# dkohlsdorf/audio_pattern_discovery

Hardware: AMD Instinct MI355X
Metric: DTW cell-updates/sec (whole node) (higher is better)
Workload: dtype f32

## Files before the change

### audio_pattern_discovery_amd/csrc/apd_internal.h

```cpp
#pragma once
#include <hip/hip_runtime.h>
#include <stdint.h>

#include <iterator>
#include <map>
#include <set>
#include <string>
#include <type_traits>
#include <utility>
#include <vector>

#include "../../include/apd.h"

struct apd_context;
namespace apd {

constexpr int kTile = 16;
constexpr int kSlotsPerTile = kTile * kTile;
constexpr int kWave = 64;

struct BandSpec {
    float pct;
    uint32_t explicit_band;
    int use_explicit;
    float ins, del, mat;
};

struct AlignLaunch {
    const float *d_frames;
    uint32_t frames_bytes;
    const uint32_t *d_seq_off;
    const float *d_seq_nmax;
    const uint4 *d_tiles;
    uint32_t n_tiles;
    uint32_t n_seq;
    uint32_t dim, dpad;
    BandSpec band;
    float *d_slab;
    const uint32_t *d_nonfinite;
    uint32_t w_max;
    uint32_t n_max;
    int variant;
    int hybrid;
    int strict;
    float tau;
};

constexpr int kKernelDims[] = {8, 10, 13, 16, 20, 26};
constexpr bool is_kernel_dim(uint32_t d) { for (int k : kKernelDims) if ((uint32_t)k == d) return true; return false; }
constexpr uint32_t kernel_dim(uint32_t d) { for (int k : kKernelDims) if ((uint32_t)k >= d) return (uint32_t)k; return d; }
constexpr int max_cells_per_lane(uint32_t d) { return d <= 13 ? 9 : (d <= 16 ? 7 : 5); }
constexpr int max_strip_columns(uint32_t d) { return d <= 10 ? 13 : (d <= 13 ? 11 : max_cells_per_lane(d)); }

struct KernelGeom {
    enum Family : uint8_t { Generic, Systolic, Wide, Strip, BandedStrip, SharedColumns };
    Family family = Generic;
    uint8_t lanes_or_waves = 0;
    uint8_t cells = 0;

    constexpr int encode() const
    {
        constexpr int base[] = {0, 0, 10000, 20000, 30000, 40000};
        return family == Generic ? 0 : base[family] + lanes_or_waves * 100 + cells;
    }
    static constexpr KernelGeom decode(int key)
    {
        const Family f = key >= 100 && key < 10000 ? Systolic : key >= 10000 && key < 20000 ? Wide
                       : key >= 20000 && key < 30000 ? Strip : key >= 30000 && key < 40000 ? BandedStrip
                       : key >= 40000 && key < 50000 ? SharedColumns : Generic;
        if (f == Generic) return KernelGeom{};
        return KernelGeom{f, (uint8_t)((key % 10000) / 100), (uint8_t)(key % 100)};
    }
    constexpr uint32_t lanes_per_pair() const
    {
        return family == Systolic || family == SharedColumns ? lanes_or_waves : family == Wide ? 64u * lanes_or_waves : 64u;
    }
    constexpr uint32_t capacity() const { return (family == Wide ? 64u : 1u) * lanes_or_waves * cells; }
    constexpr bool operator==(KernelGeom o) const { return family == o.family && lanes_or_waves == o.lanes_or_waves && cells == o.cells; }
    constexpr bool operator<(KernelGeom o) const { return encode() < o.encode(); }
};

#define APD_SYSTOLIC_GEOMS(X) X(8, 5) X(8, 7) X(8, 9) X(16, 2) X(16, 3) X(16, 5) X(16, 7) X(16, 9) X(32, 5) X(32, 7) X(32, 9) \
                              X(64, 3) X(64, 5) X(64, 7) X(64, 9)
#define APD_WIDE_GEOMS(X) X(2, 5) X(2, 7) X(2, 9) X(4, 5) X(4, 7) X(4, 9) X(8, 5) X(8, 7) X(8, 9)
#define APD_STRIP_GEOMS(X) X(1, 3) X(1, 5) X(1, 7) X(1, 9) X(1, 11) X(1, 13) X(2, 3) X(2, 5) X(2, 7) X(2, 9) X(2, 11) X(2, 13) \
                           X(4, 3) X(4, 5) X(4, 7) X(4, 9) X(4, 11) X(4, 13)
#define APD_BANDED_STRIP_GEOMS(X) X(1, 5) X(1, 9) X(4, 5) X(4, 9)
#define APD_SHARED_COLUMN_GEOMS(X) X(16, 9)

#define APD_SYSTOLIC_ENTRY_(A, B) KernelGeom{KernelGeom::Systolic, A, B},
#define APD_WIDE_ENTRY_(A, B) KernelGeom{KernelGeom::Wide, A, B},
#define APD_STRIP_ENTRY_(A, B) KernelGeom{KernelGeom::Strip, A, B},
#define APD_BANDED_STRIP_ENTRY_(A, B) KernelGeom{KernelGeom::BandedStrip, A, B},
#define APD_SHARED_COLUMN_ENTRY_(A, B) KernelGeom{KernelGeom::SharedColumns, A, B},
constexpr KernelGeom kSystolicGeoms[] = {APD_SYSTOLIC_GEOMS(APD_SYSTOLIC_ENTRY_)};
constexpr KernelGeom kWideGeoms[] = {APD_WIDE_GEOMS(APD_WIDE_ENTRY_)};
constexpr KernelGeom kStripGeoms[] = {APD_STRIP_GEOMS(APD_STRIP_ENTRY_)};
constexpr KernelGeom kBandedStripGeoms[] = {APD_BANDED_STRIP_GEOMS(APD_BANDED_STRIP_ENTRY_)};
constexpr KernelGeom kSharedColumnGeoms[] = {APD_SHARED_COLUMN_GEOMS(APD_SHARED_COLUMN_ENTRY_)};
#undef APD_SYSTOLIC_ENTRY_
#undef APD_WIDE_ENTRY_
#undef APD_STRIP_ENTRY_
#undef APD_BANDED_STRIP_ENTRY_
#undef APD_SHARED_COLUMN_ENTRY_

template <class F, size_t... I>
bool with_kernel_dim_(uint32_t dim, F &&f, std::index_sequence<I...>)
{
    return ((dim == (uint32_t)kKernelDims[I] ? (f(std::integral_constant<int, kKernelDims[I]>{}), true) : false) || ...);
}
template <class F>
bool with_kernel_dim(uint32_t dim, F &&f) { return with_kernel_dim_(dim, f, std::make_index_sequence<std::size(kKernelDims)>{}); }

constexpr bool geom_instantiated(KernelGeom g, uint32_t dim)
{
    if (g.family == KernelGeom::Generic) return true;
    if (!is_kernel_dim(dim)) return false;
    const bool strip = g.family == KernelGeom::Strip;
    if (g.cells > (strip ? max_strip_columns(dim) : max_cells_per_lane(dim))) return false;
    auto on = [g](const auto &list) { for (KernelGeom e : list) if (e == g) return true; return false; };
    return g.family == KernelGeom::Systolic ? on(kSystolicGeoms) : g.family == KernelGeom::Wide ? on(kWideGeoms)
         : g.family == KernelGeom::SharedColumns ? on(kSharedColumnGeoms) : strip ? on(kStripGeoms) : on(kBandedStripGeoms);
}
template <size_t N>
constexpr bool geoms_round_trip(const KernelGeom (&list)[N])
{
    for (KernelGeom g : list) if (!(KernelGeom::decode(g.encode()) == g)) return false;
    return true;
}
static_assert(geoms_round_trip(kSystolicGeoms) && geoms_round_trip(kWideGeoms) && geoms_round_trip(kStripGeoms) &&
                  geoms_round_trip(kBandedStripGeoms) && geoms_round_trip(kSharedColumnGeoms), "a listed geometry has no integer code of its own");

__host__ __device__ constexpr int sweep_result_offset(int rows, int cols, int w) { return (cols - 1) - (rows - 1) + w; }
__host__ __device__ constexpr int sweep_capture_step(int rows, int cols, int w, int c)
{
    return (rows - 1) + sweep_result_offset(rows, cols, w) / c;
}
__host__ __device__ constexpr int sweep_steps_needed(int rows, int cols, int w, int c) { return sweep_capture_step(rows, cols, w, c) + 1; }
static_assert(sweep_result_offset(1000, 1024, 66) == 90 && sweep_capture_step(1000, 1024, 66, 9) == 1009 &&
                  sweep_steps_needed(1000, 1024, 66, 9) == 1010, "cfg 3's shape, rows the shorter sequence: lane 10 ends the sweep");
static_assert(sweep_steps_needed(1024, 1000, 66, 9) == 1028, "the same pair with the longer sequence as rows: u* = 42, lane 4");
static_assert(sweep_capture_step(40, 72, 34, 9) == 39 + 7 && (2 * 34 + 1 + 8) / 9 == 8,
              "|n - m| = w - 2: u* = 2w - 2 sits in the last active lane, nothing is cut at the end");
static_assert(sweep_steps_needed(2, 2, 2, 2) == 3 && sweep_steps_needed(72, 40, 34, 9) == 72, "smallest pair; u* = 2: lane 0");

constexpr int shared_column_unroll(int c) { return (c + 1) % 2 == 0 ? c + 1 : 2 * (c + 1); }
constexpr int shared_column_ring_min(int g, int c) { return (g - 1) * (c - 1) + 1 + 2 * shared_column_unroll(c); }
constexpr int shared_column_ring_frames(int g, int c) { return (shared_column_ring_min(g, c) + 16 + 7) / 8 * 8; }
constexpr uint32_t shared_column_slack(KernelGeom g)
{
    return (uint32_t)(shared_column_ring_frames(g.lanes_or_waves, g.cells) - shared_column_ring_min(g.lanes_or_waves, g.cells));
}
inline uint32_t host_w(const BandSpec &b, uint32_t n, uint32_t m);
inline bool shared_columns_qualify(const std::vector<uint32_t> &lens, uint32_t tile_a, uint32_t tile_b, const BandSpec &band,
                                   uint32_t slack)
{
    const uint32_t n_seq = (uint32_t)lens.size();
    for (uint32_t sa = 0; sa < (uint32_t)kTile; sa += 4)
        for (uint32_t sb = 0; sb < (uint32_t)kTile; sb += 4) {
            uint32_t lo = 0xFFFFFFFFu, hi = 0;
            for (uint32_t i = 0; i < 16; ++i) {
                const uint32_t a = tile_a * kTile + sa + i / 4, b = tile_b * kTile + sb + i % 4;
                if (!(a < b && b < n_seq) || lens[a] < 2 || lens[b] < 2) continue;
                const uint32_t w = host_w(band, lens[a], lens[b]);
                lo = w < lo ? w : lo;
                hi = w > hi ? w : hi;
            }
            if (hi > lo && hi - lo > slack) return false;
        }
    return true;
}

constexpr uint64_t strip_lds_bytes(uint32_t dim, uint32_t ppw, bool banded, uint32_t rows)
{
    const uint64_t dp = (dim + 4) & ~3u;
    return 4 * ((ppw == 1 ? 128 : 64) * dp + (uint64_t)ppw * (banded ? 2 : 1) * (rows + 4) + 16);
}

constexpr uint32_t kPathMaxOffsets = 20480;
__host__ __device__ constexpr uint32_t path_cells_per_lane(uint32_t w) { return (2 * w + 1 + 63) / 64 < 2 ? 2u : (2 * w + 1 + 63) / 64; }
inline uint64_t path_dir_words(uint32_t n, uint32_t m, uint32_t w)
{
    if (n < 2 || m < 2) return 0;
    return ((uint64_t)n + 63) * ((path_cells_per_lane(w) + 15) / 16) * 64;
}
struct PathPair {
    uint32_t px, py;
    uint64_t dir_off;
    uint64_t step_off;
};
struct PathLaunch {
    const float *d_frames;
    const uint32_t *d_seq_off;
    uint32_t dim, dpad;
    BandSpec band;
    const PathPair *d_pairs;
    uint32_t n_pairs;
    uint32_t *d_dirs;
    apd_path_step *d_steps;
    uint32_t *d_len;
    float *d_scores;
};
hipError_t launch_path_sweep(const PathLaunch &L, uint32_t c_max, hipStream_t stream);
hipError_t launch_path_trace(const PathLaunch &L, hipStream_t stream);

constexpr uint32_t kSpotMaxQuery = 16384;
constexpr uint32_t kSpotMaxStream = 0xFFFF0000u;
constexpr uint32_t kSpotRegisterRows = 4;
constexpr uint32_t spot_rows_per_lane(uint32_t n) { return (n + 63) / 64; }
constexpr uint32_t spot_row_class(uint32_t dim, uint32_t n)
{
    return is_kernel_dim(dim) && spot_rows_per_lane(n) <= kSpotRegisterRows ? spot_rows_per_lane(n) : 0u;
}
struct SpotPair {
    uint32_t px, py;
    uint32_t out;
    uint32_t pad;
    uint64_t curve_off;
};
struct SpotLaunch {
    const float *d_frames;
    const uint32_t *d_seq_off;
    uint32_t dim, dpad;
    float ins, del, mat;
    const SpotPair *d_pairs;
    uint32_t n_pairs;
    float *d_cost;
    uint32_t *d_start;
    apd_spot_best *d_best;
};
size_t spot_lds_bytes(uint32_t rows_per_lane);
hipError_t launch_spot(const SpotLaunch &L, uint32_t rt, uint32_t r_max, hipStream_t stream);

hipError_t launch_align(const AlignLaunch &L, KernelGeom g, hipStream_t stream, std::string &err, int *status);
hipError_t launch_generic_fallback(const AlignLaunch &L, hipStream_t stream, bool *fits);
bool generic_fallback_fits(uint32_t w_max);

struct TileClass { KernelGeom geom; uint32_t first, count, w_max, n_max; };
void plan_tile_classes(const std::vector<uint64_t> &offsets, uint32_t n_seq, const std::vector<uint2> &tiles, const BandSpec &band,
                       uint32_t dim, int variant, bool fast_ok, bool uniform_pen, bool fast_shift, std::vector<TileClass> &classes,
                       std::vector<uint4> &flat);
hipError_t launch_pad(const float *d_src, float *d_dst, const uint32_t *d_seq_off, const uint32_t *d_src_off, uint32_t n_seq,
                      uint64_t n_frames_padded, uint32_t src_dim, uint32_t dim, uint32_t dpad, uint32_t *d_flags, float *d_seq_nmax,
                      hipStream_t stream);
hipError_t launch_unpack(const float *d_gathered, float *d_out, const uint32_t *d_order, uint32_t n_seq, uint32_t world,
                         uint64_t slab_floats, const uint32_t *d_flags, uint32_t *d_status, hipStream_t stream);
hipError_t launch_selftest(int *d_result, hipStream_t stream);
hipError_t launch_join_flags(uint32_t *d_flags_out, const uint32_t *d_flags_a, const uint32_t *d_flags_b, hipStream_t stream);
hipError_t launch_unpack_cross(const float *d_slab, float *d_fs, float *d_sf, const uint32_t *d_order, uint32_t n_seq, uint32_t n0,
                               uint32_t n_first, bool swapped, const uint32_t *d_flags, uint32_t *d_status, hipStream_t stream);
hipError_t launch_cross_linkage(const float *d_fs, const float *d_sf, uint32_t n_first, uint32_t n_second, const uint32_t *d_members,
                                const uint32_t *d_set_off, uint32_t n_sets, float *d_link, uint32_t *d_nearest, float *d_nearest_linkage,
                                hipStream_t stream);
hipError_t launch_sqrt_sweep(uint32_t first, uint64_t count, unsigned long long *d_out, hipStream_t stream);
constexpr float kFeatureFloor = 0x1p-40f;
constexpr float kFeatureBound = 0x1p60f;

struct DeviceBuf {
    void *ptr = nullptr;
    size_t bytes = 0;
    DeviceBuf() = default;
    DeviceBuf(DeviceBuf &&o) noexcept : ptr(o.ptr), bytes(o.bytes) { o.ptr = nullptr; o.bytes = 0; }
    DeviceBuf &operator=(DeviceBuf &&o) noexcept { std::swap(ptr, o.ptr); std::swap(bytes, o.bytes); return *this; }
    ~DeviceBuf() { reset(); }
    hipError_t reset() { const hipError_t e = ptr ? hipFree(ptr) : hipSuccess; ptr = nullptr; bytes = 0; return e; }
    hipError_t alloc(size_t n)
    {
        if (hipError_t e = reset(); e != hipSuccess) return e;
        if (hipError_t e = hipMalloc(&ptr, n); e != hipSuccess) { ptr = nullptr; return e; }
        bytes = n;
        return hipSuccess;
    }
    hipError_t reserve(size_t n) { return ptr && bytes >= n ? hipSuccess : alloc(n); }
    template <class T> T *as() const { return static_cast<T *>(ptr); }
    explicit operator bool() const { return ptr != nullptr; }
};

struct ContextChild {
    apd_context *ctx = nullptr;
    virtual void release_device() = 0;
    virtual ~ContextChild() = default;
};
int destroy_child(ContextChild *child);

int device_select(apd_context *ctx, const float *d_x, uint64_t len, uint64_t k, float *value);
uint64_t percentile_index(uint64_t len, float perc);

inline uint32_t host_band_from_pct(float pct, uint32_t len)
{
    float p = pct * (float)len;
    if (!(p > 0.0f)) return 0;
    if (p >= 4294967040.0f) return 0xFFFFFFFFu;
    return (uint32_t)p;
}
inline uint32_t host_w(const BandSpec &b, uint32_t n, uint32_t m)
{
    uint32_t mx = n > m ? n : m, gap = n > m ? n - m : m - n;
// ... 85 lines not shown
```

### audio_pattern_discovery_amd/csrc/dtw_systolic.h

```cpp
#pragma once
#include <type_traits>

#ifndef APD_ABLATE
#define APD_ABLATE 0
#endif

#include "dtw_common.h"

namespace apd {

typedef float apd_f32x4 __attribute__((ext_vector_type(4)));
constexpr uint32_t kNoFrame = 0xFFFFFF00u;

template <int D>
__device__ __forceinline__ void load_frame(float (&dst)[D], __amdgpu_buffer_rsrc_t rsrc, uint32_t byte_off)
{
    constexpr int DP4 = (D + 3) / 4;
#pragma unroll
    for (int q = 0; q < DP4; ++q) {
        const apd_f32x4 t = __builtin_bit_cast(apd_f32x4, __builtin_amdgcn_raw_buffer_load_b128(rsrc, byte_off + 16u * q, 0, 0));
        if (4 * q + 0 < D) dst[4 * q + 0] = t.x;
        if (4 * q + 1 < D) dst[4 * q + 1] = t.y;
        if (4 * q + 2 < D) dst[4 * q + 2] = t.z;
        if (4 * q + 3 < D) dst[4 * q + 3] = t.w;
// ... 255 lines not shown
            const apd_f32x4 t = *reinterpret_cast<const apd_f32x4 *>(p + 4 * q);
            if (4 * q + 0 < DN) dst[4 * q + 0] = t.x;
            if (4 * q + 1 < DN) dst[4 * q + 1] = t.y;
            if (4 * q + 2 < DN) dst[4 * q + 2] = t.z;
            if (4 * q + 3 < DN) dst[4 * q + 3] = t.w;
        }
    };
    constexpr int NX = HYBRID ? 1 : 2;
    float xs[NX][DN];
    read_row(xs[0], 0 - gl);
#pragma unroll
    for (int k = 0; k < DN; ++k) xs[NX - 1][k] = (NX == 1) ? xs[0][k] : 0.0f;
    constexpr bool PIPE = (APD_ABLATE & 32) != 0;
    float dn[C];
#pragma unroll
    for (int c = 0; c < C; ++c) dn[c] = (PIPE && !HYBRID && c < C - 1) ? frame_dist_strict<D, DN>(xs[0], yf[c]) : 0.0f;

    auto advance_window = [&](int q) __attribute__((always_inline)) {
        const int r = q % S, e = (r + C) % S;
#pragma unroll
        for (int k = 0; k < (HYBRID ? DN : D); ++k) {
            if (APD_ABLATE & 4) { yf[e][k] = yf[(r + 1) % S][k] + yf[e][k]; continue; }
            yf[e][k] = MASKED_FETCH ? dpp_move<(G == 8) ? 0x101 : 0x130>(yf[(r + 1) % S][k], yf[e][k])
                                    : group_from_upper<G>(yf[(r + 1) % S][k], yf[e][k], gl);
        }
    };
    auto macro_steps = [&](int tau_begin, int tau_end, auto slow_tag) __attribute__((always_inline)) {
        constexpr bool SLOW = decltype(slow_tag)::value;
        uint32_t yo_cur = kNoFrame, yo_cap = kNoFrame, yo_step = 0u;
        if (!SLOW && gl == G - 1) {
            yo_cap = b_off + (uint32_t)(m - 1) * FB;
            yo_cur = min(b_off + (uint32_t)(tau_begin + ((HYBRID && !MASKED_FETCH) ? 1 : 0) + (C - 1) * G - w) * FB, yo_cap);
            yo_step = FB;
        }
        auto fetch_column = [&](float (&dst)[DN], int t) __attribute__((always_inline)) {
            if (APD_ABLATE & 8) return;
            if (SLOW) {
                const int jt = t + 1 + (C - 1) * G - w;
                const uint32_t yo = b_off + (uint32_t)((jt >= 1) ? (min(jt, m) - 1) : (HYBRID ? m : m + 1)) * FB;
                load_frame<DN>(dst, rsrc, gl == G - 1 ? yo : kNoFrame);
            } else {
                load_frame<DN>(dst, rsrc, yo_cur);
                yo_cur = min(yo_cur + yo_step, yo_cap);
            }
        };
        for (int tau0 = tau_begin; tau0 < tau_end; tau0 += U) {
            apd_f32x4 fill_regs[NFILL];
            fill_load(tau0 + U + 1, fill_regs);
            const float *const xrows = &xring[((tau0 + 1 - gl) & (R - 1)) * RS];
#pragma unroll
            for (int q = 0; q < U; ++q) {
                const int tau = tau0 + q;
                const int r = q % S;
                const int xa = HYBRID ? 0 : (q & 1), xb = HYBRID ? 0 : (xa ^ 1);
                const int e = (r + C) % S;
                if (!HYBRID) {
                    fetch_column(yf[e], tau);
                    read_row_at(xs[xb], xrows + q * RS);
                }
                float d[C];
                if (HYBRID) {
#pragma unroll
                    for (int c = 0; c < C; ++c) {
                        d[c] = frame_sq_expanded_pre<D>(xs[xa], yf[(r + c) % S]);
                    }
                    float dmin = d[0];
#pragma unroll
                    for (int c = 1; c + 1 < C; c += 2) dmin = __builtin_fminf(__builtin_fminf(dmin, d[c]), d[c + 1]);
                    if (C % 2 == 0) dmin = __builtin_fminf(dmin, d[C - 1]);
                    const bool any = (APD_ABLATE & 128) ? false : dmin < (xs[xa][D] + nmax_b) * tau_thr;
                    advance_window(q);
                    if (MASKED_FETCH) {
                        if (gl == G - 1) fetch_column(yf[e], tau);
                    }
                    if (__builtin_expect(__ballot(any) != 0ull, 0)) {
                        float nx = xs[xa][D];
                        asm volatile("" : "+v"(nx));
#pragma unroll
                        for (int c = 0; c < C; ++c) {
                            const float sc = nx + yf[(r + c) % S][D];
                            const float ex = frame_sq_exact_pre<D>(xs[xa], yf[(r + c) % S]);
                            d[c] = (d[c] < sc * tau_thr) ? ex : d[c];
                        }
                    }
                    if (!MASKED_FETCH) fetch_column(yf[r], tau + 1);
#pragma unroll
                    for (int c = 0; c < C; ++c) d[c] = (APD_ABLATE & 1) ? d[c] : __builtin_amdgcn_sqrtf(d[c]);
                    read_row_at(xs[0], xrows + q * RS);
                } else if (UNIFORM_PEN && !SLOW && !PIPE) {
                    float d2[C];
#pragma unroll
                    for (int c = 0; c < C; ++c) d2[c] = frame_sq_strict<D, DN>(xs[xa], yf[(r + c) % S]);
                    float dmin = d2[0];
#pragma unroll
                    for (int c = 1; c + 1 < C; c += 2) dmin = __builtin_fminf(__builtin_fminf(dmin, d2[c]), d2[c + 1]);
                    if (C % 2 == 0) dmin = __builtin_fminf(dmin, d2[C - 1]);
                    if (__builtin_expect(__ballot(!(dmin >= 0x1p-96f)) != 0ull, 0)) {
#pragma unroll
                        for (int c = 0; c < C; ++c) d[c] = __builtin_sqrtf(d2[c]);
                    } else {
#pragma unroll
                        for (int c = 0; c < C; ++c) d[c] = sqrt_rn_finite(d2[c]);
                    }
                } else {
#pragma unroll
                    for (int c = 0; c < C; ++c)
                        d[c] = (UNIFORM_PEN && PIPE && c < C - 1) ? dn[c] : frame_dist_strict<D, DN>(xs[xa], yf[(r + c) % S]);
                    if (PIPE) {
#pragma unroll
                        for (int c = 0; c < C - 1; ++c) dn[c] = frame_dist_strict<D, DN>(xs[xb], yf[(r + 1 + c) % S]);
                    }
                }
                dp_rows_step<C, G, UNIFORM_PEN>(prev1, prev2, d, g1, g2, del, ins, mat, gl);
                if (SLOW) slow_phase_captures<C>(prev1, prev2, res1, res2, tau, gl, tau_cap, cw, cstar);
                if (!HYBRID) advance_window(q);
            }
            fill_store(tau0 + U + 1, fill_regs);
            asm volatile("" ::: "memory");
        }
    };
    macro_steps(0, a_end, std::true_type{});
    macro_steps(a_end, b_end, std::false_type{});
    macro_steps(b_end, total_r, std::true_type{});

    if (P.valid && gl == (sweep ? ustar / C : 0)) {
        if (sweep) {
            const float denom = (float)(n + m);
            store_pair_rows_b(L, tile, P, res1 / denom, res2 / denom);
        } else {
            const float s = (P.n == 1 && P.m == 1) ? 0.0f : APD_INF;
            store_pair(L, tile, P, s, s);
        }
    }
}

typedef float apd_f32x2 __attribute__((ext_vector_type(2)));
template <int DN>
__device__ __forceinline__ void read_frame_lds(float (&dst)[DN], const float *p)
{
    constexpr int FULL = DN / 4, TAIL = DN % 4;
#pragma unroll
    for (int k = 0; k < FULL; ++k) {
        const apd_f32x4 t = *reinterpret_cast<const apd_f32x4 *>(p + 4 * k);
        dst[4 * k + 0] = t.x; dst[4 * k + 1] = t.y; dst[4 * k + 2] = t.z; dst[4 * k + 3] = t.w;
    }
    if (TAIL >= 2) {
        const apd_f32x2 t = *reinterpret_cast<const apd_f32x2 *>(p + 4 * FULL);
        dst[4 * FULL + 0] = t.x; dst[4 * FULL + 1] = t.y;
    }
    if (TAIL == 1) dst[4 * FULL] = p[4 * FULL];
    if (TAIL == 3) dst[4 * FULL + 2] = p[4 * FULL + 2];
}

constexpr int shared_column_ring_floats(int rc, int u, int dp) { return (((rc + u) * dp + ((rc + u + 7) / 8) * 4) * 4 + 255) / 256 * 64; }

template <int D, int C, int G>
__global__ __launch_bounds__(256) void dtw_fused_systolic_shared(const AlignLaunch L)
{
    static_assert(C >= 2 && G == 16, "one ring per wavefront: four lane groups");
    if (L.d_nonfinite != nullptr && *L.d_nonfinite != 0u) return;
    constexpr int DN = D + 1;
    constexpr int DP = (DN + 3) & ~3;
    constexpr int PPW = 64 / G;
    constexpr int WPT = kSlotsPerTile / (4 * PPW);
    constexpr int S = C + 1;
    constexpr int U = shared_column_unroll(C);
    constexpr int RC = shared_column_ring_frames(G, C);
    constexpr int R = 64;
    constexpr int LPF = DP / 4;
    constexpr int FPF = 64 / LPF;
    constexpr int RS = DP + 4;
    constexpr uint32_t FB = DP * 4u;
    constexpr int XRING = (R + U) * RS;
    constexpr int CRING = shared_column_ring_floats(RC, U, DP);
    static_assert(FPF >= U && RC % 8 == 0, "one wave-wide load per fill");
    static_assert(RC >= (G - 1) * (C - 1) + 2 * U + (int)shared_column_slack(KernelGeom{KernelGeom::SharedColumns, G, C}),
                  "ring too short for the spread of w the tile plan admits");
    extern __shared__ __attribute__((aligned(16))) float apd_shared_lds[];
    const int lane = threadIdx.x & 63, wave = threadIdx.x >> 6;
    const int gl = lane % G;
    float *const xring = apd_shared_lds + wave * XRING;
    float *const crings = apd_shared_lds + 4 * XRING;
    int *const wg_words = reinterpret_cast<int *>(crings + PPW * CRING);
    const uint32_t xcd = blockIdx.x & 7u, q = blockIdx.x >> 3;
    const uint32_t tile = (q / WPT) * 8u + xcd;
    const uint32_t sub = q % WPT;
    const uint32_t slot = ((sub % 4u) * 4u + wave) * kTile + (sub / 4u) * 4u + lane / G;
    const PairInfo P = decode_pair_rows_b(L, tile, slot);
    const bool special = P.valid && (P.n == 1 || P.m == 1);
    const bool sweep = P.valid && !special;
    const int n = sweep ? P.n : 1, m = sweep ? P.m : 1, w = sweep ? P.w : 2;
    const int u0 = C * gl;
    const int two_w = 2 * w;
    int w_bound = w;
    asm volatile("" : "+v"(w_bound));
    int my_total = sweep ? sweep_steps_needed(n, m, w_bound, C) : 0;
    int my_min = sweep ? (n - 1) : 0x7fffffff;
    int my_w = sweep ? w : 0x7fffffff;
    int total = 0, min_rows = 0x7fffffff, w_lo = 0x7fffffff;
#pragma unroll
    for (int g = 0; g < PPW; ++g) {
        total = max(total, __builtin_amdgcn_readlane(my_total, g * G));
        min_rows = min(min_rows, __builtin_amdgcn_readlane(my_min, g * G));
        w_lo = min(w_lo, __builtin_amdgcn_readlane(my_w, g * G));
    }
    if (lane == 0) { wg_words[2 * wave] = total; wg_words[2 * wave + 1] = w_lo; }
    __syncthreads();
    total = 0; w_lo = 0x7fffffff;
#pragma unroll
    for (int k = 0; k < 4; ++k) { total = max(total, wg_words[2 * k]); w_lo = min(w_lo, wg_words[2 * k + 1]); }
    if (total == 0) {
        if (special && gl == 0) { const float s = (P.n == 1 && P.m == 1) ? 0.0f : APD_INF; store_pair(L, tile, P, s, s); }
        return;
    }
    const __amdgpu_buffer_rsrc_t rsrc = __builtin_amdgcn_make_buffer_rsrc((void *)L.d_frames, 0, L.frames_bytes, 0x00020000);
    const uint32_t a_off = (uint32_t)(P.A - L.d_frames) * 4u, b_off = (uint32_t)(P.B - L.d_frames) * 4u;
    float ins = L.band.ins, del = L.band.del, mat = L.band.mat;
    float tau_thr = L.tau, nmax_b = P.nmax_b;
    asm volatile("" : "+v"(ins), "+v"(del), "+v"(mat), "+v"(tau_thr), "+v"(nmax_b));
    const unsigned long long sweeping = __ballot(sweep);
    const int lead = sweeping ? __builtin_ctzll(sweeping) : 0;
    const uint32_t a_off_w = sweeping ? __builtin_amdgcn_readlane(a_off, lead) : 0u;
    const int n_w = sweeping ? __builtin_amdgcn_readlane(n, lead) : 1;
    uint32_t cb_off = 0u;
    int cm = 0;
    bool cvalid = false;
    {
        const uint4 t = L.d_tiles[tile];
        const uint32_t a = t.x * kTile + (sub / 4u) * 4u + wave;
        if (a < L.n_seq) {
            const uint32_t oa = L.d_seq_off[a];
            cm = (int)(L.d_seq_off[a + 1] - oa) - 2;
            cb_off = oa * L.dpad * 4u;
            cvalid = true;
        }
    }

    bool g1[C], g2[C];
#pragma unroll
    for (int c = 0; c < C; ++c) {
        const int u = u0 + c;
        g1[c] = u >= two_w;
        g2[c] = (u == 0) | (u > two_w);
    }
    const int cw = w - u0;
    const int ustar = sweep_result_offset(n, m, w);
    const int cstar = ustar - u0;
    const int tau_cap = (n - 1) + gl;
    const int total_r = ((total + U - 1) / U) * U;
    const int a_end = min(((G + U - 1) / U) * U, total_r);
    const int b_end = min(max((min_rows / U) * U, a_end), total_r);

    float prev1[C], prev2[C];
#pragma unroll
    for (int c = 0; c < C; ++c) { prev1[c] = APD_INF; prev2[c] = APD_INF; }
    float res1 = 0.0f, res2 = 0.0f;

    float yf[S][DN];
#pragma unroll
    for (int c = 0; c < C; ++c) {
        const int j = u0 - gl + c - w;
        const int idx = (j >= 1) ? (min(j, m) - 1) : m;
        load_frame<DN>(yf[c], rsrc, b_off + (uint32_t)idx * FB);
    }
#pragma unroll
    for (int k = 0; k < DN; ++k) yf[C][k] = 0.0f;

    constexpr int NFILL = (U + FPF - 1) / FPF;
    const int fill_f = lane / LPF, fill_q = lane % LPF;
    const bool fill_act = (fill_f < FPF) & (fill_f < U);
    auto fill_load = [&](int first_row, apd_f32x4 (&regs)[NFILL]) __attribute__((always_inline)) {
        const uint32_t off = a_off_w + (uint32_t)(min(first_row + fill_f, n_w) - 1) * FB + 16u * fill_q;
        regs[0] = __builtin_bit_cast(apd_f32x4, __builtin_amdgcn_raw_buffer_load_b128(rsrc, fill_act ? off : kNoFrame, 0, 0));
    };
    auto fill_store = [&](int first_row, const apd_f32x4 (&regs)[NFILL]) __attribute__((always_inline)) {
        if (fill_act) {
            apd_f32x4 v = regs[0];
            prescale_row_piece<D>(v, fill_q);
            const int rslot = (first_row + fill_f) & (R - 1);
            *reinterpret_cast<apd_f32x4 *>(&xring[rslot * RS + 4 * fill_q]) = v;
            if (rslot < U) *reinterpret_cast<apd_f32x4 *>(&xring[(rslot + R) * RS + 4 * fill_q]) = v;
        }
    };
    for (int e = lane; e < G * DP; e += 64) {
        const int rslot = (-(e / DP)) & (R - 1);
        const float v = (e % DP) == D ? APD_INF : 0.0f;
        xring[rslot * RS + (e % DP)] = v;
        if (rslot < U) xring[(rslot + R) * RS + (e % DP)] = v;
    }
    {
        apd_f32x4 regs[NFILL];
        fill_load(1, regs);
        fill_store(1, regs);
    }
    float *const cring_fill = crings + wave * CRING;
    const int col_hi0 = U + (C - 1) * G - w_lo;
    auto ring_slot = [](int j) { return (j + 64 * RC) % RC; };
    auto ring_at = [](auto *ring, uint32_t p) { return ring + p * DP + ((p >> 3) << 2); };
    auto col_load = [&](int j, bool act) __attribute__((always_inline)) {
        const int idx = (j >= 1) ? (min(j, cm) - 1) : cm;
        const uint32_t off = cb_off + (uint32_t)idx * FB + 16u * fill_q;
        return __builtin_bit_cast(apd_f32x4, __builtin_amdgcn_raw_buffer_load_b128(rsrc, (act & cvalid) ? off : kNoFrame, 0, 0));
    };
    for (int j0 = col_hi0 - RC + 1; j0 <= col_hi0; j0 += FPF) {
        const int j = j0 + fill_f;
        const bool act = (fill_f < FPF) & (j <= col_hi0);
        const apd_f32x4 v = col_load(j, act);
        const uint32_t ps = (uint32_t)ring_slot(j);
        if (act) *reinterpret_cast<apd_f32x4 *>(ring_at(cring_fill, ps) + 4 * fill_q) = v;
        if (act && ps < (uint32_t)U) *reinterpret_cast<apd_f32x4 *>(ring_at(cring_fill, ps + RC) + 4 * fill_q) = v;
    }
    uint32_t pf = (uint32_t)ring_slot(col_hi0 + 1 + fill_f);
    const float *const cring_read = crings + (lane / G) * CRING;
    uint32_t pr = (uint32_t)ring_slot(1 + (C - 1) * (gl + 1) - w);
    auto read_col = [&](float (&dst)[DN], const float *block_base, int q) __attribute__((always_inline)) {
        read_frame_lds<DN>(dst, block_base + q * DP + (((pr + (uint32_t)q) >> 3) << 2));
    };
    __syncthreads();
    auto read_row_at = [&](float (&dst)[DN], const float *p) __attribute__((always_inline)) { read_frame_lds<DN>(dst, p); };
    float xs[DN];
    read_row_at(xs, &xring[((0 - gl) & (R - 1)) * RS]);

    auto macro_steps = [&](int tau_begin, int tau_end, auto slow_tag) __attribute__((always_inline)) {
        constexpr bool SLOW = decltype(slow_tag)::value;
        for (int tau0 = tau_begin; tau0 < tau_end; tau0 += U) {
            apd_f32x4 fill_regs[NFILL];
            fill_load(tau0 + U + 1, fill_regs);
            const apd_f32x4 col_regs = col_load(tau0 + col_hi0 + 1 + fill_f, fill_act);
            const float *const xrows = &xring[((tau0 + 1 - gl) & (R - 1)) * RS];
            const float *const ycols = cring_read + pr * DP;
#pragma unroll
            for (int q = 0; q < U; ++q) {
                const int tau = tau0 + q;
                const int r = q % S;
                const int e = (r + C) % S;
                float d[C];
#pragma unroll
                for (int c = 0; c < C; ++c) d[c] = frame_sq_expanded_pre<D>(xs, yf[(r + c) % S]);
                float dmin = d[0];
#pragma unroll
                for (int c = 1; c + 1 < C; c += 2) dmin = __builtin_fminf(__builtin_fminf(dmin, d[c]), d[c + 1]);
                if (C % 2 == 0) dmin = __builtin_fminf(dmin, d[C - 1]);
                const bool any = dmin < (xs[D] + nmax_b) * tau_thr;
                read_col(yf[e], ycols, q);
                if (__builtin_expect(__ballot(any) != 0ull, 0)) {
                    float nx = xs[D];
                    asm volatile("" : "+v"(nx));
#pragma unroll
                    for (int c = 0; c < C; ++c) {
                        const float sc = nx + yf[(r + c) % S][D];
                        const float ex = frame_sq_exact_pre<D>(xs, yf[(r + c) % S]);
                        d[c] = (d[c] < sc * tau_thr) ? ex : d[c];
                    }
                }
#pragma unroll
                for (int c = 0; c < C; ++c) d[c] = __builtin_amdgcn_sqrtf(d[c]);
                read_row_at(xs, xrows + q * RS);
                dp_rows_step<C, G, true>(prev1, prev2, d, g1, g2, del, ins, mat, gl);
                if (SLOW) slow_phase_captures<C>(prev1, prev2, res1, res2, tau, gl, tau_cap, cw, cstar);
            }
            fill_store(tau0 + U + 1, fill_regs);
            if (fill_act) *reinterpret_cast<apd_f32x4 *>(ring_at(cring_fill, pf) + 4 * fill_q) = col_regs;
            if (fill_act && pf < (uint32_t)U) *reinterpret_cast<apd_f32x4 *>(ring_at(cring_fill, pf + RC) + 4 * fill_q) = col_regs;
            pf = min(pf + (uint32_t)U, pf + (uint32_t)U - (uint32_t)RC);
            pr = min(pr + (uint32_t)U, pr + (uint32_t)U - (uint32_t)RC);
            __syncthreads();
        }
    };
    macro_steps(0, a_end, std::true_type{});
    macro_steps(a_end, b_end, std::false_type{});
    macro_steps(b_end, total_r, std::true_type{});

    if (P.valid && gl == (sweep ? ustar / C : 0)) {
        if (sweep) {
            const float denom = (float)(n + m);
            store_pair_rows_b(L, tile, P, res1 / denom, res2 / denom);
        } else {
            const float s = (P.n == 1 && P.m == 1) ? 0.0f : APD_INF;
            store_pair(L, tile, P, s, s);
        }
    }
}

template <int D, int C, int G>
constexpr size_t shared_columns_lds_bytes()
{
    constexpr int DP = (D + 1 + 3) & ~3, U = shared_column_unroll(C), RC = shared_column_ring_frames(G, C);
    constexpr int XRING = (64 + U) * (DP + 4), CRING = shared_column_ring_floats(RC, U, DP);
    return (size_t)(4 * XRING + (64 / G) * CRING + 8) * sizeof(float);
}
template <int D, int C, int G>
static hipError_t launch_shared_columns_kernel(const AlignLaunch &L, hipStream_t stream)
{
    constexpr int WPT = kSlotsPerTile / (4 * (64 / G));
    constexpr size_t lds = shared_columns_lds_bytes<D, C, G>();
    static_assert(lds <= 80 * 1024, "two workgroups per CU");
    static bool granted[64] = {};
    int dev = 0;
    if (hipError_t e = hipGetDevice(&dev); e != hipSuccess) return e;
    if (dev < 0 || dev >= 64 || !granted[dev]) {
        const hipError_t e = hipFuncSetAttribute(reinterpret_cast<const void *>(dtw_fused_systolic_shared<D, C, G>),
                                                 hipFuncAttributeMaxDynamicSharedMemorySize, (int)lds);
        if (e != hipSuccess) return e;
        if (dev >= 0 && dev < 64) granted[dev] = true;
    }
    const uint32_t tiles8 = (L.n_tiles + 7u) / 8u * 8u;
    hipLaunchKernelGGL((dtw_fused_systolic_shared<D, C, G>), dim3(tiles8 * WPT), dim3(256), lds, stream, L);
    return hipSuccess;
}

template <int D, int C, int G, bool UNIFORM_PEN, bool HYBRID>
static void launch_systolic_kernel(const AlignLaunch &L, hipStream_t stream)
{
    constexpr int PPW = 64 / G;
    constexpr int WPT = kSlotsPerTile / (4 * PPW);
    const uint32_t tiles8 = (L.n_tiles + 7u) / 8u * 8u;
    hipLaunchKernelGGL((dtw_fused_systolic<D, C, G, UNIFORM_PEN, HYBRID>), dim3(tiles8 * WPT), dim3(256), 0, stream, L);
}

#ifdef APD_SYSTOLIC_STRICT_UNIT
template <int D>
bool launch_systolic_strict(const AlignLaunch &L, KernelGeom g, hipStream_t stream)
{
#define APD_CASE(GG, CC) if constexpr (geom_instantiated(KernelGeom{KernelGeom::Systolic, GG, CC}, D)) { \
        if (g == KernelGeom{KernelGeom::Systolic, GG, CC}) { launch_systolic_kernel<D, CC, GG, true, false>(L, stream); return true; } }
    APD_SYSTOLIC_GEOMS(APD_CASE)
#undef APD_CASE
    return false;
}
#else
template <int D>
bool launch_systolic(const AlignLaunch &L, KernelGeom g, hipStream_t stream)
{
    const bool unit = L.band.ins == 1.0f && L.band.del == 1.0f && L.band.mat == 1.0f;
    if (g.family == KernelGeom::SharedColumns) {
        if (!(unit && L.hybrid)) return false;
#define APD_CASE(GG, CC) if constexpr (geom_instantiated(KernelGeom{KernelGeom::SharedColumns, GG, CC}, D)) { \
        if (g == KernelGeom{KernelGeom::SharedColumns, GG, CC}) return launch_shared_columns_kernel<D, CC, GG>(L, stream) == hipSuccess; }
        APD_SHARED_COLUMN_GEOMS(APD_CASE)
#undef APD_CASE
        return false;
    }
    if (unit && !L.hybrid) return launch_systolic_strict<D>(L, g, stream);
#define APD_CASE(GG, CC) if constexpr (geom_instantiated(KernelGeom{KernelGeom::Systolic, GG, CC}, D)) { \
        if (g == KernelGeom{KernelGeom::Systolic, GG, CC}) { \
            if (!unit) launch_systolic_kernel<D, CC, GG, false, false>(L, stream); else launch_systolic_kernel<D, CC, GG, true, true>(L, stream); \
            return true; } }
    APD_SYSTOLIC_GEOMS(APD_CASE)
#undef APD_CASE
    return false;
}
#endif

}
```

Measured before the change: 3211 billion.

## Stage gate threshold in row ring, tighten slow phases, exit tail early

The fill step now precomputes the pruning gate threshold (row norm plus the wave-wide max column norm, times tau) and stores it in the spare float after each row's norm. The inner loop reads it with the row instead of doing an add and multiply per step. The slow capture head and tail phases are resized from the band width and the earliest capture step, so more macro-steps run the cheaper steady path. The tail loop can also return mid-block once all groups have passed their total. The wave-wide max norm gives a looser gate than the per-pair norm, so the exact distance path may run more often. The mid-block early return calls __syncthreads inside divergent-looking code, which is a synchronisation risk.

```diff
diff --git a/audio_pattern_discovery_amd/csrc/apd_internal.h b/audio_pattern_discovery_amd/csrc/apd_internal.h
--- a/audio_pattern_discovery_amd/csrc/apd_internal.h
+++ b/audio_pattern_discovery_amd/csrc/apd_internal.h
@@ -143,6 +143,14 @@
 static_assert(sweep_capture_step(40, 72, 34, 9) == 39 + 7 && (2 * 34 + 1 + 8) / 9 == 8,
               "|n - m| = w - 2: u* = 2w - 2 sits in the last active lane, nothing is cut at the end");
 static_assert(sweep_steps_needed(2, 2, 2, 2) == 3 && sweep_steps_needed(72, 40, 34, 9) == 72, "smallest pair; u* = 2: lane 0");
+__host__ __device__ constexpr int sweep_head_steps(int w, int c, int u) { return ((w / c) / u + 1) * u; }
+__host__ __device__ constexpr int sweep_tail_begin(int first_capture, int u) { return (first_capture / u) * u; }
+static_assert(sweep_head_steps(63, 9, 10) == 10 && sweep_head_steps(66, 9, 10) == 10 && sweep_head_steps(71, 9, 10) == 10,
+              "G C = 144 offsets hold w <= 71: 63 / 9 = 66 / 9 = 71 / 9 = 7, lane 7 injects in macro-step 7 of block 0");
+static_assert(sweep_head_steps(89, 9, 10) == 10 && sweep_head_steps(90, 9, 10) == 20 && sweep_head_steps(2, 9, 10) == 10,
+              "w = 90: lane 10 at macro-step 10, the first of block 1; an idle group (w = 2): lane 0 at macro-step 0");
+static_assert(sweep_tail_begin(1009, 10) == 1000 && sweep_tail_begin(1000, 10) == 1000 && sweep_tail_begin(999, 10) == 990,
+              "cfg 3's pair above is captured at 1009, in the block that starts at 1000");
 
 constexpr int shared_column_unroll(int c) { return (c + 1) % 2 == 0 ? c + 1 : 2 * (c + 1); }
 constexpr int shared_column_ring_min(int g, int c) { return (g - 1) * (c - 1) + 1 + 2 * shared_column_unroll(c); }
diff --git a/audio_pattern_discovery_amd/csrc/dtw_systolic.h b/audio_pattern_discovery_amd/csrc/dtw_systolic.h
--- a/audio_pattern_discovery_amd/csrc/dtw_systolic.h
+++ b/audio_pattern_discovery_amd/csrc/dtw_systolic.h
@@ -431,6 +431,32 @@
     if (TAIL == 3) dst[4 * FULL + 2] = p[4 * FULL + 2];
 }
 
+typedef float apd_f32x3 __attribute__((ext_vector_type(3)));
+template <int DN>
+__device__ __forceinline__ void read_row_frame_thr(float (&dst)[DN], float &thr, const float *p)
+{
+    constexpr int N = DN + 1, FULL = N / 4, TAIL = N % 4;
+    float t[N];
+#pragma unroll
+    for (int k = 0; k < FULL; ++k) {
+        const apd_f32x4 v = *reinterpret_cast<const apd_f32x4 *>(p + 4 * k);
+        t[4 * k + 0] = v.x; t[4 * k + 1] = v.y; t[4 * k + 2] = v.z; t[4 * k + 3] = v.w;
+    }
+    if (TAIL == 3) {
+        apd_f32x3 v;
+        __builtin_memcpy(&v, __builtin_assume_aligned(p + 4 * FULL, 16), 12);
+        t[4 * FULL + 0] = v.x; t[4 * FULL + 1] = v.y; t[4 * FULL + 2] = v.z;
+    }
+    if (TAIL == 2) {
+        const apd_f32x2 v = *reinterpret_cast<const apd_f32x2 *>(p + 4 * FULL);
+        t[4 * FULL + 0] = v.x; t[4 * FULL + 1] = v.y;
+    }
+    if (TAIL == 1) t[4 * FULL] = p[4 * FULL];
+#pragma unroll
+    for (int k = 0; k < DN; ++k) dst[k] = t[k];
+    thr = t[DN];
+}
+
 constexpr int shared_column_ring_floats(int rc, int u, int dp) { return (((rc + u) * dp + ((rc + u + 7) / 8) * 4) * 4 + 255) / 256 * 64; }
 
 template <int D, int C, int G>
@@ -453,6 +479,7 @@
     constexpr int XRING = (R + U) * RS;
     constexpr int CRING = shared_column_ring_floats(RC, U, DP);
     static_assert(FPF >= U && RC % 8 == 0, "one wave-wide load per fill");
+    static_assert(DN < DP, "the row slot has no spare float behind the norm for the staged gate threshold");
     static_assert(RC >= (G - 1) * (C - 1) + 2 * U + (int)shared_column_slack(KernelGeom{KernelGeom::SharedColumns, G, C}),
                   "ring too short for the spread of w the tile plan admits");
     extern __shared__ __attribute__((aligned(16))) float apd_shared_lds[];
@@ -474,14 +501,17 @@
     int w_bound = w;
     asm volatile("" : "+v"(w_bound));
     int my_total = sweep ? sweep_steps_needed(n, m, w_bound, C) : 0;
-    int my_min = sweep ? (n - 1) : 0x7fffffff;
+    int my_cap = sweep ? my_total - 1 : 0x7fffffff;
     int my_w = sweep ? w : 0x7fffffff;
-    int total = 0, min_rows = 0x7fffffff, w_lo = 0x7fffffff;
+    int total = 0, first_cap = 0x7fffffff, w_lo = 0x7fffffff, w_hi = 2;
+    float nmax_w = 0.0f;
 #pragma unroll
     for (int g = 0; g < PPW; ++g) {
         total = max(total, __builtin_amdgcn_readlane(my_total, g * G));
-        min_rows = min(min_rows, __builtin_amdgcn_readlane(my_min, g * G));
+        first_cap = min(first_cap, __builtin_amdgcn_readlane(my_cap, g * G));
         w_lo = min(w_lo, __builtin_amdgcn_readlane(my_w, g * G));
+        w_hi = max(w_hi, __builtin_amdgcn_readlane(w, g * G));
+        nmax_w = fmaxf(nmax_w, __builtin_bit_cast(float, __builtin_amdgcn_readlane(__builtin_bit_cast(int, P.nmax_b), g * G)));
     }
     if (lane == 0) { wg_words[2 * wave] = total; wg_words[2 * wave + 1] = w_lo; }
     __syncthreads();
@@ -495,8 +525,8 @@
     const __amdgpu_buffer_rsrc_t rsrc = __builtin_amdgcn_make_buffer_rsrc((void *)L.d_frames, 0, L.frames_bytes, 0x00020000);
     const uint32_t a_off = (uint32_t)(P.A - L.d_frames) * 4u, b_off = (uint32_t)(P.B - L.d_frames) * 4u;
     float ins = L.band.ins, del = L.band.del, mat = L.band.mat;
-    float tau_thr = L.tau, nmax_b = P.nmax_b;
-    asm volatile("" : "+v"(ins), "+v"(del), "+v"(mat), "+v"(tau_thr), "+v"(nmax_b));
+    float tau_thr = L.tau;
+    asm volatile("" : "+v"(ins), "+v"(del), "+v"(mat), "+v"(tau_thr));
     const unsigned long long sweeping = __ballot(sweep);
     const int lead = sweeping ? __builtin_ctzll(sweeping) : 0;
     const uint32_t a_off_w = sweeping ? __builtin_amdgcn_readlane(a_off, lead) : 0u;
@@ -527,8 +557,8 @@
     const int cstar = ustar - u0;
     const int tau_cap = (n - 1) + gl;
     const int total_r = ((total + U - 1) / U) * U;
-    const int a_end = min(((G + U - 1) / U) * U, total_r);
-    const int b_end = min(max((min_rows / U) * U, a_end), total_r);
+    const int a_end = min(sweep_head_steps(w_hi, C, U), total_r);
+    const int b_end = min(max(sweep_tail_begin(first_cap, U), a_end), total_r);
 
     float prev1[C], prev2[C];
 #pragma unroll
@@ -556,6 +586,11 @@
         if (fill_act) {
             apd_f32x4 v = regs[0];
             prescale_row_piece<D>(v, fill_q);
+            if (fill_q == D / 4) {
+                if (D % 4 == 0) v.y = (v.x + nmax_w) * tau_thr;
+                if (D % 4 == 1) v.z = (v.y + nmax_w) * tau_thr;
+                if (D % 4 == 2) v.w = (v.z + nmax_w) * tau_thr;
+            }
             const int rslot = (first_row + fill_f) & (R - 1);
             *reinterpret_cast<apd_f32x4 *>(&xring[rslot * RS + 4 * fill_q]) = v;
             if (rslot < U) *reinterpret_cast<apd_f32x4 *>(&xring[(rslot + R) * RS + 4 * fill_q]) = v;
@@ -563,7 +598,7 @@
     };
     for (int e = lane; e < G * DP; e += 64) {
         const int rslot = (-(e / DP)) & (R - 1);
-        const float v = (e % DP) == D ? APD_INF : 0.0f;
+        const float v = ((e % DP) == D || (e % DP) == DN) ? APD_INF : 0.0f;
         xring[rslot * RS + (e % DP)] = v;
         if (rslot < U) xring[(rslot + R) * RS + (e % DP)] = v;
     }
@@ -596,12 +631,16 @@
         read_frame_lds<DN>(dst, block_base + q * DP + (((pr + (uint32_t)q) >> 3) << 2));
     };
     __syncthreads();
-    auto read_row_at = [&](float (&dst)[DN], const float *p) __attribute__((always_inline)) { read_frame_lds<DN>(dst, p); };
-    float xs[DN];
+    float xs[DN], thr;
+    auto read_row_at = [&](float (&dst)[DN], const float *p) __attribute__((always_inline)) { read_row_frame_thr<DN>(dst, thr, p); };
     read_row_at(xs, &xring[((0 - gl) & (R - 1)) * RS]);
 
-    auto macro_steps = [&](int tau_begin, int tau_end, auto slow_tag) __attribute__((always_inline)) {
-        constexpr bool SLOW = decltype(slow_tag)::value;
+    using Steady = std::integral_constant<int, 0>;
+    using SlowHead = std::integral_constant<int, 1>;
+    using SlowTail = std::integral_constant<int, 2>;
+    auto macro_steps = [&](int tau_begin, int tau_end, auto phase) __attribute__((always_inline)) {
+        constexpr bool SLOW = decltype(phase)::value != 0;
+        constexpr bool BOUNDED = decltype(phase)::value == 2;
         for (int tau0 = tau_begin; tau0 < tau_end; tau0 += U) {
             apd_f32x4 fill_regs[NFILL];
             fill_load(tau0 + U + 1, fill_regs);
@@ -613,6 +652,7 @@
                 const int tau = tau0 + q;
                 const int r = q % S;
                 const int e = (r + C) % S;
+                if (BOUNDED && q > 0 && tau >= total) { __syncthreads(); return; }
                 float d[C];
 #pragma unroll
                 for (int c = 0; c < C; ++c) d[c] = frame_sq_expanded_pre<D>(xs, yf[(r + c) % S]);
@@ -620,7 +660,7 @@
 #pragma unroll
                 for (int c = 1; c + 1 < C; c += 2) dmin = __builtin_fminf(__builtin_fminf(dmin, d[c]), d[c + 1]);
                 if (C % 2 == 0) dmin = __builtin_fminf(dmin, d[C - 1]);
-                const bool any = dmin < (xs[D] + nmax_b) * tau_thr;
+                const bool any = dmin < thr;
                 read_col(yf[e], ycols, q);
                 if (__builtin_expect(__ballot(any) != 0ull, 0)) {
                     float nx = xs[D];
@@ -646,9 +686,9 @@
             __syncthreads();
         }
     };
-    macro_steps(0, a_end, std::true_type{});
-    macro_steps(a_end, b_end, std::false_type{});
-    macro_steps(b_end, total_r, std::true_type{});
+    macro_steps(0, a_end, SlowHead{});
+    macro_steps(a_end, b_end, Steady{});
+    macro_steps(b_end, total_r, SlowTail{});
 
     if (P.valid && gl == (sweep ? ustar / C : 0)) {
         if (sweep) {
```

After: 3227 billion (median of 6 runs). No clear change (+0.5%).

## Start systolic sweep at first band step and exit early at last needed step

Applied to the files above, without the earlier changes.

When all pairs in a workgroup share the same band class, the shared-column kernel now begins the anti-diagonal sweep at the first step where the origin cell enters the lanes, instead of at step zero. The prologue loads, ring pointers and initial DP state are shifted to match. The kernel also leaves the final slow phase as soon as the last needed step is reached, rather than rounding up to a full unroll block. Together these skip leading and trailing sweep steps that only process inactive band cells, at the cost of extra shared-memory words, a wider reduction of band widths, and more delicate ring-offset bookkeeping.

```diff
diff --git a/audio_pattern_discovery_amd/csrc/apd_internal.h b/audio_pattern_discovery_amd/csrc/apd_internal.h
--- a/audio_pattern_discovery_amd/csrc/apd_internal.h
+++ b/audio_pattern_discovery_amd/csrc/apd_internal.h
@@ -143,6 +143,10 @@
 static_assert(sweep_capture_step(40, 72, 34, 9) == 39 + 7 && (2 * 34 + 1 + 8) / 9 == 8,
               "|n - m| = w - 2: u* = 2w - 2 sits in the last active lane, nothing is cut at the end");
 static_assert(sweep_steps_needed(2, 2, 2, 2) == 3 && sweep_steps_needed(72, 40, 34, 9) == 72, "smallest pair; u* = 2: lane 0");
+__host__ __device__ constexpr int sweep_first_step(int w, int c) { return w / c + 1; }
+static_assert(sweep_first_step(66, 9) == 8 && sweep_first_step(2, 9) == 1, "cfg 3's band: lane 7 holds the origin; the smallest band: lane 0");
+static_assert(sweep_first_step(62, 9) == 7 && sweep_first_step(63, 9) == 8 && sweep_first_step(71, 9) == 8,
+              "w = 63 .. 71 is one class (lane 7); 71 is the widest band G C = 144 offsets hold");
 
 constexpr int shared_column_unroll(int c) { return (c + 1) % 2 == 0 ? c + 1 : 2 * (c + 1); }
 constexpr int shared_column_ring_min(int g, int c) { return (g - 1) * (c - 1) + 1 + 2 * shared_column_unroll(c); }
diff --git a/audio_pattern_discovery_amd/csrc/dtw_systolic.h b/audio_pattern_discovery_amd/csrc/dtw_systolic.h
--- a/audio_pattern_discovery_amd/csrc/dtw_systolic.h
+++ b/audio_pattern_discovery_amd/csrc/dtw_systolic.h
@@ -453,6 +453,7 @@
     constexpr int XRING = (R + U) * RS;
     constexpr int CRING = shared_column_ring_floats(RC, U, DP);
     static_assert(FPF >= U && RC % 8 == 0, "one wave-wide load per fill");
+    static_assert(G / 2 <= U, "a late start (sweep_first_step <= G / 2: G C >= 2w + 1) within two fills of the row ring's prologue");
     static_assert(RC >= (G - 1) * (C - 1) + 2 * U + (int)shared_column_slack(KernelGeom{KernelGeom::SharedColumns, G, C}),
                   "ring too short for the spread of w the tile plan admits");
     extern __shared__ __attribute__((aligned(16))) float apd_shared_lds[];
@@ -474,20 +475,29 @@
     int w_bound = w;
     asm volatile("" : "+v"(w_bound));
     int my_total = sweep ? sweep_steps_needed(n, m, w_bound, C) : 0;
-    int my_min = sweep ? (n - 1) : 0x7fffffff;
+    int my_cap = sweep ? my_total - 1 : 0x7fffffff;
     int my_w = sweep ? w : 0x7fffffff;
-    int total = 0, min_rows = 0x7fffffff, w_lo = 0x7fffffff;
+    int my_w_hi = sweep ? w : 0;
+    int total = 0, min_cap = 0x7fffffff, w_lo = 0x7fffffff, w_hi = 0;
 #pragma unroll
     for (int g = 0; g < PPW; ++g) {
         total = max(total, __builtin_amdgcn_readlane(my_total, g * G));
-        min_rows = min(min_rows, __builtin_amdgcn_readlane(my_min, g * G));
+        min_cap = min(min_cap, __builtin_amdgcn_readlane(my_cap, g * G));
         w_lo = min(w_lo, __builtin_amdgcn_readlane(my_w, g * G));
-    }
-    if (lane == 0) { wg_words[2 * wave] = total; wg_words[2 * wave + 1] = w_lo; }
+        w_hi = max(w_hi, __builtin_amdgcn_readlane(my_w_hi, g * G));
+    }
+    if (lane == 0) { wg_words[3 * wave] = total; wg_words[3 * wave + 1] = w_lo; wg_words[3 * wave + 2] = w_hi; }
     __syncthreads();
-    total = 0; w_lo = 0x7fffffff;
-#pragma unroll
-    for (int k = 0; k < 4; ++k) { total = max(total, wg_words[2 * k]); w_lo = min(w_lo, wg_words[2 * k + 1]); }
+    total = 0; w_lo = 0x7fffffff; w_hi = 0;
+#pragma unroll
+    for (int k = 0; k < 4; ++k) {
+        total = max(total, wg_words[3 * k]);
+        w_lo = min(w_lo, wg_words[3 * k + 1]);
+        w_hi = max(w_hi, wg_words[3 * k + 2]);
+    }
+    total = __builtin_amdgcn_readfirstlane(total);
+    w_lo = __builtin_amdgcn_readfirstlane(w_lo);
+    w_hi = __builtin_amdgcn_readfirstlane(w_hi);
     if (total == 0) {
         if (special && gl == 0) { const float s = (P.n == 1 && P.m == 1) ? 0.0f : APD_INF; store_pair(L, tile, P, s, s); }
         return;
@@ -526,19 +536,25 @@
     const int ustar = sweep_result_offset(n, m, w);
     const int cstar = ustar - u0;
     const int tau_cap = (n - 1) + gl;
-    const int total_r = ((total + U - 1) / U) * U;
-    const int a_end = min(((G + U - 1) / U) * U, total_r);
-    const int b_end = min(max((min_rows / U) * U, a_end), total_r);
+    const int tau_s = sweep_first_step(w_lo, C) == sweep_first_step(w_hi, C) ? sweep_first_step(w_lo, C) : 0;
+    const int total_r = tau_s + ((total - tau_s + U - 1) / U) * U;
+    min_cap = min(min_cap, total - 1);
+    const int a_end = tau_s > 0 ? tau_s : min(((G + U - 1) / U) * U, total_r);
+    const int b_end = min(max(tau_s + ((min_cap - tau_s) / U) * U, a_end), total_r);
 
     float prev1[C], prev2[C];
 #pragma unroll
     for (int c = 0; c < C; ++c) { prev1[c] = APD_INF; prev2[c] = APD_INF; }
+    if (tau_s > 0) {
+#pragma unroll
+        for (int c = 0; c < C; ++c) if (c == cw) { prev1[c] = 0.0f; prev2[c] = 0.0f; }
+    }
     float res1 = 0.0f, res2 = 0.0f;
 
     float yf[S][DN];
 #pragma unroll
     for (int c = 0; c < C; ++c) {
-        const int j = u0 - gl + c - w;
+        const int j = tau_s + u0 - gl + c - w;
         const int idx = (j >= 1) ? (min(j, m) - 1) : m;
         load_frame<DN>(yf[c], rsrc, b_off + (uint32_t)idx * FB);
     }
@@ -571,9 +587,14 @@
         apd_f32x4 regs[NFILL];
         fill_load(1, regs);
         fill_store(1, regs);
+        if (tau_s > 0) {
+            fill_load(tau_s + 1, regs);
+            fill_store(tau_s + 1, regs);
+        }
     }
     float *const cring_fill = crings + wave * CRING;
     const int col_hi0 = U + (C - 1) * G - w_lo;
+    const int col_hi_s = tau_s + col_hi0;
     auto ring_slot = [](int j) { return (j + 64 * RC) % RC; };
     auto ring_at = [](auto *ring, uint32_t p) { return ring + p * DP + ((p >> 3) << 2); };
     auto col_load = [&](int j, bool act) __attribute__((always_inline)) {
@@ -581,24 +602,24 @@
         const uint32_t off = cb_off + (uint32_t)idx * FB + 16u * fill_q;
         return __builtin_bit_cast(apd_f32x4, __builtin_amdgcn_raw_buffer_load_b128(rsrc, (act & cvalid) ? off : kNoFrame, 0, 0));
     };
-    for (int j0 = col_hi0 - RC + 1; j0 <= col_hi0; j0 += FPF) {
+    for (int j0 = col_hi_s - RC + 1; j0 <= col_hi_s; j0 += FPF) {
         const int j = j0 + fill_f;
-        const bool act = (fill_f < FPF) & (j <= col_hi0);
+        const bool act = (fill_f < FPF) & (j <= col_hi_s);
         const apd_f32x4 v = col_load(j, act);
         const uint32_t ps = (uint32_t)ring_slot(j);
         if (act) *reinterpret_cast<apd_f32x4 *>(ring_at(cring_fill, ps) + 4 * fill_q) = v;
         if (act && ps < (uint32_t)U) *reinterpret_cast<apd_f32x4 *>(ring_at(cring_fill, ps + RC) + 4 * fill_q) = v;
     }
-    uint32_t pf = (uint32_t)ring_slot(col_hi0 + 1 + fill_f);
+    uint32_t pf = (uint32_t)ring_slot(col_hi_s + 1 + fill_f);
     const float *const cring_read = crings + (lane / G) * CRING;
-    uint32_t pr = (uint32_t)ring_slot(1 + (C - 1) * (gl + 1) - w);
+    uint32_t pr = (uint32_t)ring_slot(tau_s + 1 + (C - 1) * (gl + 1) - w);
     auto read_col = [&](float (&dst)[DN], const float *block_base, int q) __attribute__((always_inline)) {
         read_frame_lds<DN>(dst, block_base + q * DP + (((pr + (uint32_t)q) >> 3) << 2));
     };
     __syncthreads();
     auto read_row_at = [&](float (&dst)[DN], const float *p) __attribute__((always_inline)) { read_frame_lds<DN>(dst, p); };
     float xs[DN];
-    read_row_at(xs, &xring[((0 - gl) & (R - 1)) * RS]);
+    read_row_at(xs, &xring[((tau_s - gl) & (R - 1)) * RS]);
 
     auto macro_steps = [&](int tau_begin, int tau_end, auto slow_tag) __attribute__((always_inline)) {
         constexpr bool SLOW = decltype(slow_tag)::value;
@@ -637,6 +658,10 @@
                 read_row_at(xs, xrows + q * RS);
                 dp_rows_step<C, G, true>(prev1, prev2, d, g1, g2, del, ins, mat, gl);
                 if (SLOW) slow_phase_captures<C>(prev1, prev2, res1, res2, tau, gl, tau_cap, cw, cstar);
+                if (SLOW && tau + 1 >= total) {
+                    __syncthreads();
+                    return;
+                }
             }
             fill_store(tau0 + U + 1, fill_regs);
             if (fill_act) *reinterpret_cast<apd_f32x4 *>(ring_at(cring_fill, pf) + 4 * fill_q) = col_regs;
@@ -646,7 +671,7 @@
             __syncthreads();
         }
     };
-    macro_steps(0, a_end, std::true_type{});
+    macro_steps(tau_s, a_end, std::true_type{});
     macro_steps(a_end, b_end, std::false_type{});
     macro_steps(b_end, total_r, std::true_type{});
 
@@ -666,7 +691,7 @@
 {
     constexpr int DP = (D + 1 + 3) & ~3, U = shared_column_unroll(C), RC = shared_column_ring_frames(G, C);
     constexpr int XRING = (64 + U) * (DP + 4), CRING = shared_column_ring_floats(RC, U, DP);
-    return (size_t)(4 * XRING + (64 / G) * CRING + 8) * sizeof(float);
+    return (size_t)(4 * XRING + (64 / G) * CRING + 12) * sizeof(float);
 }
 template <int D, int C, int G>
 static hipError_t launch_shared_columns_kernel(const AlignLaunch &L, hipStream_t stream)
```

After: 3193 billion before, 3224 billion after, median of 6. No clear change (+1.0%).
